# yzqin/s4g-release

Measured on AMD Instinct MI355X. Metric: scenes/sec (25.6k-pt clouds) end-to-end grasp inference, higher is better.
Workload: dtype f32 (f16x2 split)

## Files before the change

### s4g_release_amd/csrc/mlp_heads.hip

```cpp
#include <stdlib.h>

#include "mlp_common.h"

#ifndef S4G_HEADS_ABLATE
#define S4G_HEADS_ABLATE 0
#endif

namespace s4g {

__device__ __forceinline__ void heads_keep_alive(const f32x16& v) { asm volatile("" ::"v"(v)); }

struct HeadsParams {
  int P, N;
  const float* X;
  int ldx;
  const uint16_t* W[5];
  const float* bias[5];
  const float* wsc[5];
  float* out[4];
  int ch[4];
  long long obs[4];
  int head_mask;
  int sigmoid_head;
  const float* a_amax;
  float a_floor;
  int rps;
  const uint16_t* Wp[2];
  const float* bias_p[2];
  const float* wsc_p[2];
  const int* nidx;
  const float* nw;
  const float* sparse;
  const float* dense;
  const float* lbias;
  const float* a_amax2;
  int N2;
};

template <int PL, int HD_RING, int NRBT, bool PRE>
__global__ __launch_bounds__(512, 2) void mlp_heads_kernel(const HeadsParams p) {
  constexpr int BM = 32 * NRBT, C = 256, NW = 8, astr = C + 8, aplane = BM * astr;
  constexpr int FB = PL * 1024;
  extern __shared__ __attribute__((aligned(16))) float smemf[];
  uint16_t* PA = reinterpret_cast<uint16_t*>(smemf);
  uint16_t* PB = PA + PL * aplane;
  float* scr = reinterpret_cast<float*>(PB + PL * aplane);

  const int t = threadIdx.x;
  const int lane = t & 63;
  const int li = lane & 31, lh = lane >> 5;
  const int wv = __builtin_amdgcn_readfirstlane(t >> 6);
  const int p0 = blockIdx.x * BM;
  const uint32_t wf_lane = (uint32_t)lane * 16u;

  float sa = 1.f, inv_sa = 1.f;
  if constexpr (PL == 2) {
    float amax = p.a_floor;
    if constexpr (PRE) {
      if (p.a_amax) amax += amax_rows(p.a_amax, lane, p0, min(p0 + BM, p.P) - 1, p.rps);
      if (p.a_amax2) amax += amax_rows(p.a_amax2, lane, p0, min(p0 + BM, p.P) - 1, p.rps);
    } else if (p.a_amax) {
      amax = fmaxf(amax, amax_rows(p.a_amax, lane, p0, min(p0 + BM, p.P) - 1, p.rps));
    }
    uint32_t ex = __float_as_uint(amax) >> 23;
    ex = ex < 15u ? 15u : (ex > 240u ? 240u : ex);
    ex = __builtin_amdgcn_readfirstlane(ex);
    sa = __uint_as_float((268u - ex) << 23);
    inv_sa = __uint_as_float((ex - 14u) << 23);
  }

  WRef wrs[5];
#pragma unroll
  for (int L = 0; L < 5; ++L) wrs[L] = wref(p.W[L], 0);
  auto woff = [&](int n32, int nks, int ks) { return (size_t)((n32 * nks + ks) * FB); };
  auto w0 = [&](int g, int h) { return wrs[0] + woff(g * 16 + h * 8 + wv, 16, 0); };
  auto w1 = [&](int g, int h) { return wrs[1] + woff(g * 8 + wv, 32, h * 16); };
  auto w2 = [&](int g) { return wrs[2] + woff(g * 8 + wv, 16, 0); };
  auto w3 = [&](int g) { return wrs[3] + woff(g * 4 + (wv & 3), 16, 0); };
  auto wl = [&](int g) { return wrs[4] + woff(g, 8, 0); };
  auto wload = [&](const WRef& w, uint32_t byte_off, int pl) { return wref_load(w, wf_lane + pl * 1024, byte_off); };
  const WRef wp0 = PRE ? wref(p.Wp[0], woff(wv, 16, 0)) : wrs[0];
  const WRef wp1 = PRE ? wref(p.Wp[1], woff(wv, 16, 0)) : wrs[0];

  const int hmask = p.head_mask;
  const int g_first = __builtin_ctz(hmask);
  uint4 ring[HD_RING][PL];
  {
    const WRef w = PRE ? wp0 : w0(g_first, 0);
#pragma unroll
    for (int d = 0; d < HD_RING; ++d)
#pragma unroll
      for (int pl = 0; pl < PL; ++pl) ring[d][pl] = wload(w, d * FB, pl);
  }

#pragma unroll 1
  for (int r0 = 0; r0 < BM; r0 += 64) {
    const int row = r0 + (t >> 3), chunk = t & 7;
    const bool ok = p0 + row < p.P;
    float4 ra[8];
    if constexpr (PRE) {
      const int pos = ok ? p0 + row : 0;
      const int bq = pos / p.N;
      int i3[3];
      float w3[3];
#pragma unroll
      for (int k = 0; k < 3; ++k) {
        i3[k] = bq * p.N2 + p.nidx[(size_t)pos * 3 + k];
        w3[k] = p.nw[(size_t)pos * 3 + k];
      }
#pragma unroll
      for (int h = 0; h < 2; ++h) {
        float4 a[4], b[4], c[4], y[4], bb[4];
#pragma unroll
        for (int kk = 0; kk < 4; ++kk) {
          const int col = (h * 4 + kk) * 32 + chunk * 4;
          a[kk] = *reinterpret_cast<const float4*>(p.sparse + (size_t)i3[0] * 256 + col);
          b[kk] = *reinterpret_cast<const float4*>(p.sparse + (size_t)i3[1] * 256 + col);
          c[kk] = *reinterpret_cast<const float4*>(p.sparse + (size_t)i3[2] * 256 + col);
          bb[kk] = *reinterpret_cast<const float4*>(p.lbias + col);
          y[kk] = p.dense ? *reinterpret_cast<const float4*>(p.dense + (size_t)pos * 256 + col)
                          : make_float4(0.f, 0.f, 0.f, 0.f);
        }
#pragma unroll
        for (int kk = 0; kk < 4; ++kk) {
          const float av[4] = {a[kk].x, a[kk].y, a[kk].z, a[kk].w}, bv[4] = {b[kk].x, b[kk].y, b[kk].z, b[kk].w};
          const float cv[4] = {c[kk].x, c[kk].y, c[kk].z, c[kk].w}, yv[4] = {y[kk].x, y[kk].y, y[kk].z, y[kk].w};
          const float bi[4] = {bb[kk].x, bb[kk].y, bb[kk].z, bb[kk].w};
          float r[4];
#pragma unroll
          for (int e = 0; e < 4; ++e) {
            float acc = __fmul_rn(av[e], w3[0]);
            acc = __fadd_rn(acc, __fmul_rn(bv[e], w3[1]));
            acc = __fadd_rn(acc, __fmul_rn(cv[e], w3[2]));
            r[e] = ok ? fmaxf(__fadd_rn(__fadd_rn(yv[e], acc), bi[e]), 0.f) : 0.f;
          }
          ra[h * 4 + kk] = make_float4(r[0], r[1], r[2], r[3]);
        }
      }
    } else {
    const float* src = p.X + (size_t)(ok ? p0 + row : 0) * p.ldx + chunk * 4;
#pragma unroll
    for (int kt = 0; kt < 8; ++kt)
      ra[kt] = ok ? nt_load4(src + kt * 32) : make_float4(0.f, 0.f, 0.f, 0.f);
    }
#pragma unroll
    for (int kt = 0; kt < 8; ++kt) {
      uint16_t* dst = PA + row * astr + kt * 32 + chunk * 4;
      if constexpr (PL == 2) {
        uint2 h, l;
        split2_h<false>(ra[kt], sa, h, l);
        *reinterpret_cast<uint2*>(dst) = h;
        *reinterpret_cast<uint2*>(dst + aplane) = l;
      } else {
        *reinterpret_cast<uint2*>(dst) = make_uint2(cvt_pk_bf16(ra[kt].x, ra[kt].y), cvt_pk_bf16(ra[kt].z, ra[kt].w));
      }
    }
  }
  __syncthreads();

#define S4G_HD_TERM(NRB, PA_, PB_, ZERO)                                                            \
  _Pragma("unroll") for (int rb = 0; rb < NRB; ++rb)                                                \
    acc[rb] = chain_mfma<PL>(bf[PB_], af[rb][PA_], (ZERO) ? zero16 : acc[rb]);
#define S4G_HD_STRIP(PANEL, NRB, ROWOFF, WCUR, NKS, WNEXT)                                          \
  {                                                                                                 \
    const uint16_t* a_lane = (PANEL) + ((ROWOFF) + li) * astr + 8 * lh;                             \
    uint4 afn[NRBT][PL];                                                                            \
    _Pragma("unroll") for (int rb = 0; rb < NRB; ++rb) _Pragma("unroll") for (int pl = 0; pl < PL; ++pl) \
      afn[rb][pl] = *reinterpret_cast<const uint4*>(a_lane + pl * aplane + rb * 32 * astr);         \
    const WRef wcur_ = (WCUR);                                                                      \
    const WRef wnext_ = (WNEXT);                                                                    \
    _Pragma("unroll") for (int ks = 0; ks < NKS; ++ks) {                                            \
      const int d = ks % HD_RING;                                                                   \
      const int ksn = ks + 1 == NKS ? 0 : ks + 1;                                                   \
      uint4 af[NRBT][PL], bf[PL];                                                                   \
      _Pragma("unroll") for (int rb = 0; rb < NRB; ++rb) _Pragma("unroll") for (int pl = 0; pl < PL; ++pl) { \
        af[rb][pl] = afn[rb][pl];                                                                   \
        if (!(S4G_HEADS_ABLATE & 2))                                                                \
          afn[rb][pl] = *reinterpret_cast<const uint4*>(a_lane + pl * aplane + rb * 32 * astr + ksn * 16); \
      }                                                                                             \
      _Pragma("unroll") for (int pl = 0; pl < PL; ++pl) bf[pl] = ring[d][pl];                       \
      {                                                                                             \
        const int kr = ks + HD_RING;                                                                \
        _Pragma("unroll") for (int pl = 0; pl < PL; ++pl)                                           \
          if (!(S4G_HEADS_ABLATE & 1))                                                              \
            ring[d][pl] = kr < NKS ? wload(wcur_, kr * FB, pl) : wload(wnext_, (kr - NKS) * FB, pl); \
      }                                                                                             \
      if constexpr (PL == 2) {                                                                      \
        S4G_HD_TERM(NRB, 0, 1, ks == 0)                                                             \
        S4G_HD_TERM(NRB, 1, 0, false)                                                               \
        S4G_HD_TERM(NRB, 0, 0, false)                                                               \
      } else {                                                                                      \
        S4G_HD_TERM(NRB, 0, 0, ks == 0)                                                             \
      }                                                                                             \
      _Pragma("unroll") for (int q = 0; q < PL; ++q) {                                              \
        __builtin_amdgcn_sched_group_barrier(0x008, 1, 0);                                          \
        __builtin_amdgcn_sched_group_barrier(0x020, 1, 0);                                          \
        __builtin_amdgcn_sched_group_barrier(0x008, 1, 0);                                          \
        __builtin_amdgcn_sched_group_barrier(0x100, 1, 0);                                          \
      }                                                                                             \
      __builtin_amdgcn_sched_barrier(0);                                                            \
    }                                                                                               \
  }

  f32x16 zero16;
#pragma unroll
  for (int r = 0; r < 16; ++r) zero16[r] = 0.f;
  f32x16 acc[NRBT];
  float* epi_s = scr + wv * 64;

  auto stage_sb2 = [&](const float* wsc, const float* bias, int gch, float mul) {
    epi_s[lane] = lane < 32 ? (PL == 2 ? mul * wsc[gch + lane] : 1.f) : bias[gch + lane - 32];
  };
  auto stage_sb = [&](int L, int gch, float mul) { stage_sb2(p.wsc[L], p.bias[L], gch, mul); };

  float inv_sh = 1.f;
  auto panel_epilogue_to = [&](uint16_t* PD, auto nrb_tag, int rowoff, int pch0) {
    constexpr int NRB = decltype(nrb_tag)::value;
    if (S4G_HEADS_ABLATE & 4) {
#pragma unroll
      for (int rb = 0; rb < NRB; ++rb) heads_keep_alive(acc[rb]);
      if (!(S4G_HEADS_ABLATE & 8)) {
        __syncthreads();
        __syncthreads();
      }
      return;
    }
    float tmax = 0.f;
#pragma unroll
    for (int j = 0; j < 4; ++j) {
      const float4 sc4 = *reinterpret_cast<const float4*>(epi_s + 8 * j + 4 * lh);
      const float4 b4 = *reinterpret_cast<const float4*>(epi_s + 32 + 8 * j + 4 * lh);
      const float scv[4] = {sc4.x, sc4.y, sc4.z, sc4.w};
      const float bv[4] = {b4.x, b4.y, b4.z, b4.w};
#pragma unroll
      for (int rb = 0; rb < NRB; ++rb) {
        const f32x2 x01 = pk_fma(f32x2{acc[rb][4 * j], acc[rb][4 * j + 1]}, f32x2{scv[0], scv[1]}, f32x2{bv[0], bv[1]});
        const f32x2 x23 = pk_fma(f32x2{acc[rb][4 * j + 2], acc[rb][4 * j + 3]}, f32x2{scv[2], scv[3]}, f32x2{bv[2], bv[3]});
        const float x[4] = {fmaxf(x01.x, 0.f), fmaxf(x01.y, 0.f), fmaxf(x23.x, 0.f), fmaxf(x23.y, 0.f)};
#pragma unroll
        for (int e = 0; e < 4; ++e) acc[rb][4 * j + e] = x[e];
        if constexpr (PL == 2) {
          tmax = fmaxf(fmaxf(tmax, x[0]), x[1]);
          tmax = fmaxf(fmaxf(tmax, x[2]), x[3]);
        }
      }
    }
    float sh = 1.f;
    if constexpr (PL == 2) {
      const uint32_t wm = wave_max_u32(__float_as_uint(tmax));
      if (lane == 0) scr[NW * 64 + wv] = __uint_as_float(wm);
    }
    __syncthreads();
    if constexpr (PL == 2) {
      float hmax = scr[NW * 64];
#pragma unroll
      for (int w = 1; w < NW; ++w) hmax = fmaxf(hmax, scr[NW * 64 + w]);
      uint32_t exh = __float_as_uint(hmax) >> 23;
      exh = exh < 15u ? 15u : (exh > 240u ? 240u : exh);
      exh = __builtin_amdgcn_readfirstlane(exh);
      sh = __uint_as_float((268u - exh) << 23);
      inv_sh = __uint_as_float((exh - 14u) << 23);
    }
#pragma unroll
    for (int j = 0; j < 4; ++j)
#pragma unroll
      for (int rb = 0; rb < NRB; ++rb) {
        uint16_t* dst = PD + (rowoff + rb * 32 + li) * astr + pch0 + 8 * j + 4 * lh;
        if constexpr (PL == 2) {
          const float4 v = make_float4(acc[rb][4 * j], acc[rb][4 * j + 1], acc[rb][4 * j + 2], acc[rb][4 * j + 3]);
          uint2 h, l;
          split2_h<false>(v, sh, h, l);
          *reinterpret_cast<uint2*>(dst) = h;
          *reinterpret_cast<uint2*>(dst + aplane) = l;
        } else {
          *reinterpret_cast<uint2*>(dst) = make_uint2(cvt_pk_bf16(acc[rb][4 * j], acc[rb][4 * j + 1]),
                                                      cvt_pk_bf16(acc[rb][4 * j + 2], acc[rb][4 * j + 3]));
        }
      }
    __syncthreads();
  };
  auto panel_epilogue = [&](auto nrb_tag, int rowoff, int pch0) { panel_epilogue_to(PB, nrb_tag, rowoff, pch0); };
  using full = std::integral_constant<int, NRBT>;
  using half = std::integral_constant<int, NRBT / 2>;

  if constexpr (PRE) {
    stage_sb2(p.wsc_p[0], p.bias_p[0], wv * 32, inv_sa);
    S4G_HD_STRIP(PA, NRBT, 0, wp0, 16, wp1)
    panel_epilogue(full{}, 0, wv * 32);
    stage_sb2(p.wsc_p[1], p.bias_p[1], wv * 32, inv_sh);
    S4G_HD_STRIP(PB, NRBT, 0, wp1, 16, w0(g_first, 0))
    panel_epilogue_to(PA, full{}, 0, wv * 32);
    inv_sa = inv_sh;
  }

  for (int g = g_first, gn; g >= 0; g = gn) {
    const int rest = hmask >> (g + 1);
    gn = rest ? g + 1 + __builtin_ctz(rest) : -1;
    const int gnx = gn >= 0 ? gn : g;
    f32x16 acc1[NRBT];
    stage_sb(0, g * 512 + wv * 32, inv_sa);
    S4G_HD_STRIP(PA, NRBT, 0, w0(g, 0), 16, w1(g, 0))
    panel_epilogue(full{}, 0, wv * 32);
    S4G_HD_STRIP(PB, NRBT, 0, w1(g, 0), 16, w0(g, 1))
#pragma unroll
    for (int rb = 0; rb < NRBT; ++rb)
#pragma unroll
      for (int r = 0; r < 16; r += 2) {
        const f32x2 v = f32x2{acc[rb][r], acc[rb][r + 1]} * f32x2{inv_sh, inv_sh};
        acc1[rb][r] = v.x;
        acc1[rb][r + 1] = v.y;
      }
    stage_sb(0, g * 512 + 256 + wv * 32, inv_sa);
    S4G_HD_STRIP(PA, NRBT, 0, w0(g, 1), 16, w1(g, 1))
    panel_epilogue(full{}, 0, wv * 32);
    S4G_HD_STRIP(PB, NRBT, 0, w1(g, 1), 16, w2(g))
#pragma unroll
    for (int rb = 0; rb < NRBT; ++rb)
#pragma unroll
      for (int r = 0; r < 16; r += 2) {
        const f32x2 v = pk_fma(f32x2{acc[rb][r], acc[rb][r + 1]}, f32x2{inv_sh, inv_sh}, f32x2{acc1[rb][r], acc1[rb][r + 1]});
        acc[rb][r] = v.x;
        acc[rb][r + 1] = v.y;
      }
    stage_sb(1, g * 256 + wv * 32, 1.f);
    panel_epilogue(full{}, 0, wv * 32);
    stage_sb(2, g * 256 + wv * 32, inv_sh);
    S4G_HD_STRIP(PB, NRBT, 0, w2(g), 16, w3(g))
    panel_epilogue(full{}, 0, wv * 32);
    {
      const int row3 = (wv >> 2) * (BM / 2), cg = wv & 3;
      stage_sb(3, g * 128 + cg * 32, inv_sh);
      const WRef after = wv < NRBT ? wl(g) : w0(gnx, 0);
      S4G_HD_STRIP(PB, NRBT / 2, row3, w3(g), 16, after)
      panel_epilogue(half{}, row3, cg * 32);
    }
    if (wv < NRBT) {
      stage_sb(4, g * 32, inv_sh);
      S4G_HD_STRIP(PB, 1, wv * 32, wl(g), 8, w0(gnx, 0))
      const int row = p0 + wv * 32 + li;
      const int b = row / p.N, pt = row - b * p.N;
      const int nch = p.ch[g];
      float* __restrict__ base = p.out[g] + (size_t)b * (size_t)p.obs[g] + pt;
#pragma unroll
      for (int j = 0; j < 4; ++j) {
        const float4 sc4 = *reinterpret_cast<const float4*>(epi_s + 8 * j + 4 * lh);
        const float4 b4 = *reinterpret_cast<const float4*>(epi_s + 32 + 8 * j + 4 * lh);
        const float scv[4] = {sc4.x, sc4.y, sc4.z, sc4.w};
        const float bv[4] = {b4.x, b4.y, b4.z, b4.w};
#pragma unroll
        for (int e = 0; e < 4; ++e) {
          const int c = 8 * j + 4 * lh + e;
          float x = __fmaf_rn(acc[0][4 * j + e], scv[e], bv[e]);
          if (g == p.sigmoid_head) x = 1.0f / (1.0f + expf(-x));
          if (c < nch && row < p.P) base[(size_t)c * p.N] = x;
        }
      }
    }
  }
#undef S4G_HD_STRIP
#undef S4G_HD_TERM
}

template <int PL, int HD_RING, int NRBT, bool PRE>
static int launch_heads_cfg(const HeadsParams& p, hipStream_t st) {
  constexpr int BM = 32 * NRBT;
  constexpr size_t lds = sizeof(uint16_t) * 2 * PL * BM * (256 + 8) + sizeof(float) * (8 * 64 + 16);
  static_assert(lds <= 160 * 1024, "one workgroup's panels must fit a CU's LDS");
  static LdsAttrCache lds_cache;
  if (int rc = allow_dynamic_lds(reinterpret_cast<const void*>(&mlp_heads_kernel<PL, HD_RING, NRBT, PRE>), lds, lds_cache)) return rc;
  hipLaunchKernelGGL((mlp_heads_kernel<PL, HD_RING, NRBT, PRE>), dim3((unsigned)((p.P + BM - 1) / BM)), dim3(512), lds, st, p);
  S4G_LAUNCH_CHECK();
  return S4G_OK;
}
template <int PL, int HD_RING, int NRBT>
static int launch_heads(const HeadsParams& p, hipStream_t st) {
  return p.Wp[0] ? launch_heads_cfg<PL, HD_RING, NRBT, true>(p, st) : launch_heads_cfg<PL, HD_RING, NRBT, false>(p, st);
}

}

extern "C" int s4g_heads_chain_f32(const s4g_heads_desc_t* d, s4g_stream_t stream) {
  using namespace s4g;
  if (!d || d->P < 0 || d->N <= 0) return S4G_EINVAL;
  const bool pre = d->pre_W_frag[0] != nullptr;
  if (!pre && (!d->X || (d->ldx & 3) || d->ldx < 256 || ((uintptr_t)d->X & 15))) return S4G_EINVAL;
  if (pre && (!d->pre_W_frag[1] || !d->pre_bias[0] || !d->pre_bias[1] || !d->pre_nidx || !d->pre_nw ||
              !d->pre_sparse || !d->pre_lbias || d->pre_N2 < 3 || ((uintptr_t)d->pre_sparse & 15) ||
              ((uintptr_t)d->pre_dense & 15) || ((uintptr_t)d->pre_lbias & 15) ||
              (d->precision == S4G_GEMM_F16X2 && (!d->pre_w_inv_scale[0] || !d->pre_w_inv_scale[1]))))
    return S4G_EINVAL;
  if (d->precision != S4G_GEMM_F16X2 && d->precision != S4G_GEMM_BF16) return S4G_EINVAL;
  if (d->C != 256 || d->H0 != 512 || d->H1 != 256 || d->H2 != 256 || d->H3 != 128) return S4G_EUNSUPPORTED;
  HeadsParams p;
  p.P = d->P;
  p.N = d->N;
  p.X = d->X;
  p.ldx = d->ldx;
  for (int l = 0; l < 5; ++l) {
    if (!d->W_frag[l] || !d->bias[l] || (d->precision == S4G_GEMM_F16X2 && !d->w_inv_scale[l])) return S4G_EINVAL;
    p.W[l] = (const uint16_t*)d->W_frag[l];
    p.bias[l] = d->bias[l];
    p.wsc[l] = d->w_inv_scale[l];
  }
  p.head_mask = d->head_mask ? d->head_mask : 15;
  if (p.head_mask < 0 || p.head_mask > 15) return S4G_EINVAL;
  for (int h = 0; h < 4; ++h) {
    p.out[h] = nullptr;
    p.ch[h] = 0;
    p.obs[h] = 0;
    if (!((p.head_mask >> h) & 1)) continue;
    if (!d->out[h] || d->channels[h] <= 0 || d->channels[h] > 32) return S4G_EINVAL;
    p.out[h] = d->out[h];
    p.ch[h] = d->channels[h];
    if (d->out_batch_stride != 0 && d->out_batch_stride < (int64_t)d->channels[h] * d->N) return S4G_EINVAL;
    p.obs[h] = d->out_batch_stride != 0 ? (long long)d->out_batch_stride : (long long)d->channels[h] * d->N;
  }
  p.sigmoid_head = d->sigmoid_head;
  p.a_amax = d->a_amax;
  p.a_floor = d->a_amax_floor;
  p.rps = d->rows_per_scene > 0 ? d->rows_per_scene : 0;
  for (int l = 0; l < 2; ++l) {
    p.Wp[l] = pre ? (const uint16_t*)d->pre_W_frag[l] : nullptr;
    p.bias_p[l] = pre ? d->pre_bias[l] : nullptr;
    p.wsc_p[l] = pre ? d->pre_w_inv_scale[l] : nullptr;
  }
  p.nidx = pre ? d->pre_nidx : nullptr;
  p.nw = pre ? d->pre_nw : nullptr;
  p.sparse = pre ? d->pre_sparse : nullptr;
  p.dense = pre ? d->pre_dense : nullptr;
  p.lbias = pre ? d->pre_lbias : nullptr;
  p.a_amax2 = pre ? d->pre_a_amax2 : nullptr;
  p.N2 = pre ? d->pre_N2 : 0;
  if (d->precision == S4G_GEMM_F16X2 && !d->a_amax && !(d->a_amax_floor > 0.f)) return S4G_EINVAL;
  if (d->P == 0) return S4G_OK;
  hipStream_t st = (hipStream_t)stream;
  if (d->precision == S4G_GEMM_F16X2) return launch_heads<2, 4, 2>(p, st);
  return launch_heads<1, 4, 4>(p, st);
}
```

Measured before the change: 2074.

## Make MLP heads kernel persistent with atomic tile queue and next-tile prefetch

Turns the heads kernel into a persistent kernel launched with one workgroup per CU, where workgroups pull tiles from a global atomic queue kept in a per-stream slot and reset by the last workgroup to finish. On the last head of each tile, the f16x2 NRBT=2 path prefetches the next tile's interpolated input and amax scale, staging it into the LDS A panel while the remaining GEMM strips run. This is meant to hide the input gather and split latency behind MFMA work and to cut per-workgroup launch and prologue overhead. In exchange it adds host-side slot bookkeeping (mutex, graph-capture handling), more register pressure, and correctness risk from the queue reset.

```diff
diff --git a/s4g_release_amd/csrc/mlp_heads.hip b/s4g_release_amd/csrc/mlp_heads.hip
--- a/s4g_release_amd/csrc/mlp_heads.hip
+++ b/s4g_release_amd/csrc/mlp_heads.hip
@@ -1,4 +1,6 @@
 #include <stdlib.h>
+
+#include <mutex>
 
 #include "mlp_common.h"
 
@@ -35,39 +37,73 @@
   const float* lbias;
   const float* a_amax2;
   int N2;
+  int ntiles, qslot;
 };
 
-template <int PL, int HD_RING, int NRBT, bool PRE>
+constexpr int HQ_EAGER = 64, HQ_SLOTS = 256;
+__device__ unsigned int g_heads_queue[HQ_SLOTS][2];
+
+#ifdef S4G_HEADS_STAMPS
+__device__ unsigned long long g_heads_stamps[512 * 8];
+#define S4G_HSTAMP(i)                                                                              \
+  do {                                                                                             \
+    const unsigned sb_ = p.ntiles >= 1024 ? (unsigned)(tile - p.ntiles / 2) : (unsigned)tile;      \
+    if (threadIdx.x == 0 && sb_ < 512u) g_heads_stamps[sb_ * 8 + (i)] = __builtin_amdgcn_s_memtime(); \
+  } while (0)
+#else
+#define S4G_HSTAMP(i)
+#endif
+
+template <int PL, int HD_RING, int NRBT, bool PRE, bool PERSIST>
 __global__ __launch_bounds__(512, 2) void mlp_heads_kernel(const HeadsParams p) {
   constexpr int BM = 32 * NRBT, C = 256, NW = 8, astr = C + 8, aplane = BM * astr;
+  constexpr bool PF = PERSIST && PL == 2 && NRBT == 2;
   constexpr int FB = PL * 1024;
   extern __shared__ __attribute__((aligned(16))) float smemf[];
   uint16_t* PA = reinterpret_cast<uint16_t*>(smemf);
   uint16_t* PB = PA + PL * aplane;
   float* scr = reinterpret_cast<float*>(PB + PL * aplane);
+  int* tile_s = reinterpret_cast<int*>(scr + NW * 64 + 8);
+  float* lb_s = scr + NW * 64 + 16;
 
   const int t = threadIdx.x;
   const int lane = t & 63;
   const int li = lane & 31, lh = lane >> 5;
   const int wv = __builtin_amdgcn_readfirstlane(t >> 6);
-  const int p0 = blockIdx.x * BM;
   const uint32_t wf_lane = (uint32_t)lane * 16u;
 
-  float sa = 1.f, inv_sa = 1.f;
-  if constexpr (PL == 2) {
+  auto fetch_tile = [&]() {
+    if (t == 0) tile_s[0] = (int)atomicAdd(&g_heads_queue[p.qslot][0], 1u);
+  };
+  int tile = blockIdx.x;
+  if constexpr (PERSIST) {
+    fetch_tile();
+    if constexpr (PF && PRE) {
+      if (t < 256) lb_s[t] = p.lbias[t];
+    }
+    __syncthreads();
+    tile = __builtin_amdgcn_readfirstlane(tile_s[0]);
+  }
+  if (!PERSIST || tile < p.ntiles) {
+  int p0 = tile * BM;
+
+  auto tile_exp = [&](int q0, bool pre, float va, float vb) -> uint32_t {
     float amax = p.a_floor;
+    const int q1 = min(q0 + BM, p.P) - 1;
+    auto rows = [&](const float* slots, float v) {
+      return pre ? __uint_as_float(wave_max_u32(__float_as_uint(v))) : amax_rows(slots, lane, q0, q1, p.rps);
+    };
     if constexpr (PRE) {
-      if (p.a_amax) amax += amax_rows(p.a_amax, lane, p0, min(p0 + BM, p.P) - 1, p.rps);
-      if (p.a_amax2) amax += amax_rows(p.a_amax2, lane, p0, min(p0 + BM, p.P) - 1, p.rps);
+      if (p.a_amax) amax += rows(p.a_amax, va);
+      if (p.a_amax2) amax += rows(p.a_amax2, vb);
     } else if (p.a_amax) {
-      amax = fmaxf(amax, amax_rows(p.a_amax, lane, p0, min(p0 + BM, p.P) - 1, p.rps));
+      amax = fmaxf(amax, rows(p.a_amax, va));
     }
     uint32_t ex = __float_as_uint(amax) >> 23;
     ex = ex < 15u ? 15u : (ex > 240u ? 240u : ex);
-    ex = __builtin_amdgcn_readfirstlane(ex);
-    sa = __uint_as_float((268u - ex) << 23);
-    inv_sa = __uint_as_float((ex - 14u) << 23);
-  }
+    return __builtin_amdgcn_readfirstlane(ex);
+  };
+  float sa = 1.f, inv_sa = 1.f;
 
   WRef wrs[5];
 #pragma unroll
@@ -84,18 +120,47 @@
 
   const int hmask = p.head_mask;
   const int g_first = __builtin_ctz(hmask);
+  const WRef w_first = PRE ? wp0 : w0(g_first, 0);
   uint4 ring[HD_RING][PL];
-  {
-    const WRef w = PRE ? wp0 : w0(g_first, 0);
-#pragma unroll
-    for (int d = 0; d < HD_RING; ++d)
-#pragma unroll
-      for (int pl = 0; pl < PL; ++pl) ring[d][pl] = wload(w, d * FB, pl);
-  }
+
+  auto interp4 = [&](const float4 a, const float4 b, const float4 c, const float4 y, const float4 bb, const float (&w3)[3], bool ok) {
+    const float av[4] = {a.x, a.y, a.z, a.w}, bv[4] = {b.x, b.y, b.z, b.w};
+    const float cv[4] = {c.x, c.y, c.z, c.w}, yv[4] = {y.x, y.y, y.z, y.w};
+    const float bi[4] = {bb.x, bb.y, bb.z, bb.w};
+    float r[4];
+#pragma unroll
+    for (int e = 0; e < 4; ++e) {
+      float acc = __fmul_rn(av[e], w3[0]);
+      acc = __fadd_rn(acc, __fmul_rn(bv[e], w3[1]));
+      acc = __fadd_rn(acc, __fmul_rn(cv[e], w3[2]));
+      r[e] = ok ? fmaxf(__fadd_rn(__fadd_rn(yv[e], acc), bi[e]), 0.f) : 0.f;
+    }
+    return make_float4(r[0], r[1], r[2], r[3]);
+  };
+
+  auto in_loop = [](int v) {
+    asm volatile("" : "+v"(v));
+    return v;
+  };
+  bool have_x = false;
+  float inv_sa_n = 1.f;
+  for (;;) {
+  S4G_HSTAMP(0);
+  if (!PF || !have_x) {
+  if constexpr (PL == 2) {
+    const uint32_t ex = tile_exp(p0, false, 0.f, 0.f);
+    sa = __uint_as_float((268u - ex) << 23);
+    inv_sa = __uint_as_float((ex - 14u) << 23);
+  }
+#pragma unroll
+  for (int d = 0; d < HD_RING; ++d)
+#pragma unroll
+    for (int pl = 0; pl < PL; ++pl) ring[d][pl] = wload(w_first, d * FB, pl);
 
 #pragma unroll 1
   for (int r0 = 0; r0 < BM; r0 += 64) {
-    const int row = r0 + (t >> 3), chunk = t & 7;
+    const int tp = PERSIST ? in_loop(t) : t;
+    const int row = r0 + (tp >> 3), chunk = tp & 7;
     const bool ok = p0 + row < p.P;
     float4 ra[8];
     if constexpr (PRE) {
@@ -122,20 +187,7 @@
                           : make_float4(0.f, 0.f, 0.f, 0.f);
         }
 #pragma unroll
-        for (int kk = 0; kk < 4; ++kk) {
-          const float av[4] = {a[kk].x, a[kk].y, a[kk].z, a[kk].w}, bv[4] = {b[kk].x, b[kk].y, b[kk].z, b[kk].w};
-          const float cv[4] = {c[kk].x, c[kk].y, c[kk].z, c[kk].w}, yv[4] = {y[kk].x, y[kk].y, y[kk].z, y[kk].w};
-          const float bi[4] = {bb[kk].x, bb[kk].y, bb[kk].z, bb[kk].w};
-          float r[4];
-#pragma unroll
-          for (int e = 0; e < 4; ++e) {
-            float acc = __fmul_rn(av[e], w3[0]);
-            acc = __fadd_rn(acc, __fmul_rn(bv[e], w3[1]));
-            acc = __fadd_rn(acc, __fmul_rn(cv[e], w3[2]));
-            r[e] = ok ? fmaxf(__fadd_rn(__fadd_rn(yv[e], acc), bi[e]), 0.f) : 0.f;
-          }
-          ra[h * 4 + kk] = make_float4(r[0], r[1], r[2], r[3]);
-        }
+        for (int kk = 0; kk < 4; ++kk) ra[h * 4 + kk] = interp4(a[kk], b[kk], c[kk], y[kk], bb[kk], w3, ok);
       }
     } else {
     const float* src = p.X + (size_t)(ok ? p0 + row : 0) * p.ldx + chunk * 4;
@@ -157,6 +209,85 @@
     }
   }
   __syncthreads();
+  } else {
+    inv_sa = inv_sa_n;
+  }
+  S4G_HSTAMP(1);
+
+  int nt = p.ntiles;
+  int n_pos = 0, n_i3[3] = {0, 0, 0};
+  bool n_ok = false, n_one = false;
+  float n_w3[3] = {0.f, 0.f, 0.f}, n_va = 0.f, n_vb = 0.f, n_sa = 1.f;
+  float4 pf[PRE ? 4 : 1][2];
+  auto pf_ids = [&]() {
+    nt = __builtin_amdgcn_readfirstlane(tile_s[0]);
+    if (nt < p.ntiles) {
+      const int q0 = nt * BM, q1 = min(q0 + BM, p.P) - 1;
+      n_ok = q0 + (t >> 3) < p.P;
+      n_pos = n_ok ? q0 + (t >> 3) : 0;
+      const int s0 = p.rps > 0 ? q0 / p.rps : 0, s1 = p.rps > 0 ? q1 / p.rps : 0;
+      n_one = s0 == s1;
+      if (n_one) {
+        if (p.a_amax) n_va = p.a_amax[(size_t)s0 * 64 + lane];
+        if (PRE && p.a_amax2) n_vb = p.a_amax2[(size_t)s0 * 64 + lane];
+      }
+      if constexpr (PRE) {
+#pragma unroll
+        for (int k = 0; k < 3; ++k) {
+          n_i3[k] = p.nidx[(size_t)n_pos * 3 + k];
+          n_w3[k] = p.nw[(size_t)n_pos * 3 + k];
+        }
+      }
+    }
+  };
+  auto pf_load = [&](int q) {
+    if (nt < p.ntiles) {
+      const int chunk = in_loop(t) & 7;
+      if (q == 0) {
+        const uint32_t ex = tile_exp(nt * BM, n_one, n_va, n_vb);
+        n_sa = __uint_as_float((268u - ex) << 23);
+        inv_sa_n = __uint_as_float((ex - 14u) << 23);
+      }
+      if constexpr (PRE) {
+        if (q == 0) {
+          const int bq = n_pos / p.N;
+#pragma unroll
+          for (int k = 0; k < 3; ++k) n_i3[k] += bq * p.N2;
+        }
+#pragma unroll
+        for (int kk = 0; kk < 2; ++kk) {
+          const int col = (q * 2 + kk) * 32 + chunk * 4;
+#pragma unroll
+          for (int k = 0; k < 3; ++k) pf[k][kk] = *reinterpret_cast<const float4*>(p.sparse + (size_t)n_i3[k] * 256 + col);
+          pf[3][kk] = p.dense ? *reinterpret_cast<const float4*>(p.dense + (size_t)n_pos * 256 + col)
+                              : make_float4(0.f, 0.f, 0.f, 0.f);
+        }
+      } else {
+        const float* src = p.X + (size_t)n_pos * p.ldx + chunk * 4;
+#pragma unroll
+        for (int kk = 0; kk < 2; ++kk)
+          pf[0][kk] = n_ok ? nt_load4(src + (q * 2 + kk) * 32) : make_float4(0.f, 0.f, 0.f, 0.f);
+      }
+    }
+  };
+  auto pf_store = [&](int q) {
+    if (nt < p.ntiles) {
+      const int tq = in_loop(t);
+      const int row = tq >> 3, chunk = tq & 7;
+#pragma unroll
+      for (int kk = 0; kk < 2; ++kk) {
+        const int col = (q * 2 + kk) * 32 + chunk * 4;
+        float4 r = pf[0][kk];
+        if constexpr (PRE)
+          r = interp4(pf[0][kk], pf[1][kk], pf[2][kk], pf[3][kk], *reinterpret_cast<const float4*>(lb_s + col), n_w3, n_ok);
+        uint16_t* dst = PA + row * astr + col;
+        uint2 hh, ll;
+        split2_h<false>(r, n_sa, hh, ll);
+        *reinterpret_cast<uint2*>(dst) = hh;
+        *reinterpret_cast<uint2*>(dst + aplane) = ll;
+      }
+    }
+  };
 
 #define S4G_HD_TERM(NRB, PA_, PB_, ZERO)                                                            \
   _Pragma("unroll") for (int rb = 0; rb < NRB; ++rb)                                                \
@@ -297,10 +428,17 @@
     const int rest = hmask >> (g + 1);
     gn = rest ? g + 1 + __builtin_ctz(rest) : -1;
     const int gnx = gn >= 0 ? gn : g;
+    const WRef w_after = PF && gn < 0 ? w_first : w0(gnx, 0);
+    if constexpr (PF) {
+      if (gn < 0) fetch_tile();
+    }
     f32x16 acc1[NRBT];
     stage_sb(0, g * 512 + wv * 32, inv_sa);
     S4G_HD_STRIP(PA, NRBT, 0, w0(g, 0), 16, w1(g, 0))
     panel_epilogue(full{}, 0, wv * 32);
+    if constexpr (PF) {
+      if (gn < 0) pf_ids();
+    }
     S4G_HD_STRIP(PB, NRBT, 0, w1(g, 0), 16, w0(g, 1))
 #pragma unroll
     for (int rb = 0; rb < NRBT; ++rb)
@@ -311,9 +449,24 @@
         acc1[rb][r + 1] = v.y;
       }
     stage_sb(0, g * 512 + 256 + wv * 32, inv_sa);
+    if constexpr (PF) {
+      if (gn < 0) pf_load(0);
+    }
     S4G_HD_STRIP(PA, NRBT, 0, w0(g, 1), 16, w1(g, 1))
     panel_epilogue(full{}, 0, wv * 32);
+    if constexpr (PF) {
+      if (gn < 0) {
+        pf_store(0);
+        pf_load(1);
+      }
+    }
     S4G_HD_STRIP(PB, NRBT, 0, w1(g, 1), 16, w2(g))
+    if constexpr (PF) {
+      if (gn < 0) {
+        pf_store(1);
+        pf_load(2);
+      }
+    }
 #pragma unroll
     for (int rb = 0; rb < NRBT; ++rb)
 #pragma unroll
@@ -326,17 +479,29 @@
     panel_epilogue(full{}, 0, wv * 32);
     stage_sb(2, g * 256 + wv * 32, inv_sh);
     S4G_HD_STRIP(PB, NRBT, 0, w2(g), 16, w3(g))
+    if (gn < 0) { S4G_HSTAMP(2); }
+    if constexpr (PF) {
+      if (gn < 0) {
+        pf_store(2);
+        pf_load(3);
+      }
+    }
     panel_epilogue(full{}, 0, wv * 32);
     {
       const int row3 = (wv >> 2) * (BM / 2), cg = wv & 3;
       stage_sb(3, g * 128 + cg * 32, inv_sh);
-      const WRef after = wv < NRBT ? wl(g) : w0(gnx, 0);
+      const WRef after = wv < NRBT ? wl(g) : w_after;
       S4G_HD_STRIP(PB, NRBT / 2, row3, w3(g), 16, after)
       panel_epilogue(half{}, row3, cg * 32);
+      if constexpr (PF) {
+        if (gn < 0) pf_store(3);
+      }
     }
     if (wv < NRBT) {
+      if (gn < 0) { S4G_HSTAMP(3); }
       stage_sb(4, g * 32, inv_sh);
-      S4G_HD_STRIP(PB, 1, wv * 32, wl(g), 8, w0(gnx, 0))
+      S4G_HD_STRIP(PB, 1, wv * 32, wl(g), 8, w_after)
+      const int lhl = PERSIST ? in_loop(lh) : lh;
       const int row = p0 + wv * 32 + li;
       const int b = row / p.N, pt = row - b * p.N;
       const int nch = p.ch[g];
@@ -349,28 +514,114 @@
         const float bv[4] = {b4.x, b4.y, b4.z, b4.w};
 #pragma unroll
         for (int e = 0; e < 4; ++e) {
-          const int c = 8 * j + 4 * lh + e;
+          const int c = 8 * j + 4 * lhl + e;
           float x = __fmaf_rn(acc[0][4 * j + e], scv[e], bv[e]);
           if (g == p.sigmoid_head) x = 1.0f / (1.0f + expf(-x));
           if (c < nch && row < p.P) base[(size_t)c * p.N] = x;
         }
       }
-    }
+      if (gn < 0) { S4G_HSTAMP(4); }
+    }
+  }
+  S4G_HSTAMP(5);
+  if constexpr (!PERSIST) {
+    break;
+  } else if constexpr (PF) {
+    if (nt >= p.ntiles) break;
+    __syncthreads();
+    tile = nt;
+    have_x = true;
+  } else {
+    fetch_tile();
+    __syncthreads();
+    tile = __builtin_amdgcn_readfirstlane(tile_s[0]);
+    if (tile >= p.ntiles) break;
+  }
+  p0 = tile * BM;
+  }
   }
 #undef S4G_HD_STRIP
 #undef S4G_HD_TERM
-}
-
-template <int PL, int HD_RING, int NRBT, bool PRE>
-static int launch_heads_cfg(const HeadsParams& p, hipStream_t st) {
+  if constexpr (PERSIST) {
+    if (t == 0) {
+      __threadfence();
+      if (atomicAdd(&g_heads_queue[p.qslot][1], 1u) == gridDim.x - 1) {
+        __threadfence();
+        atomicExch(&g_heads_queue[p.qslot][0], 0u);
+        atomicExch(&g_heads_queue[p.qslot][1], 0u);
+      }
+    }
+  }
+}
+
+struct HeadsQueueHost {
+  std::mutex m;
+  hipStream_t streams[HQ_EAGER];
+  int nstreams = 0, ncaptured = 0;
+};
+static int heads_queue_slot(hipStream_t st, int dev) {
+  static HeadsQueueHost host[64];
+  if (dev < 0 || dev >= 64) return -1;
+  hipStreamCaptureStatus cs = hipStreamCaptureStatusNone;
+  if (hipStreamIsCapturing(st, &cs) != hipSuccess) {
+    (void)hipGetLastError();
+    return -1;
+  }
+  HeadsQueueHost& h = host[dev];
+  std::lock_guard<std::mutex> lock(h.m);
+  if (cs != hipStreamCaptureStatusNone) return h.ncaptured < HQ_SLOTS - HQ_EAGER ? HQ_EAGER + h.ncaptured++ : -1;
+  for (int i = 0; i < h.nstreams; ++i)
+    if (h.streams[i] == st) return i;
+  if (h.nstreams == HQ_EAGER) return -1;
+  h.streams[h.nstreams] = st;
+  return h.nstreams++;
+}
+static int heads_cu_count(int dev) {
+  static std::atomic<int> cus[64];
+  const bool slot = dev >= 0 && dev < 64;
+  int n = slot ? cus[dev].load(std::memory_order_relaxed) : 0;
+  if (n > 0) return n;
+  if (hipDeviceGetAttribute(&n, hipDeviceAttributeMultiprocessorCount, dev) != hipSuccess || n <= 0) {
+    (void)hipGetLastError();
+    return 0;
+  }
+  if (slot) cus[dev].store(n, std::memory_order_relaxed);
+  return n;
+}
+
+template <int PL, int HD_RING, int NRBT, bool PRE, bool PERSIST>
+static int launch_heads_form(const HeadsParams& p, unsigned grid, hipStream_t st) {
   constexpr int BM = 32 * NRBT;
-  constexpr size_t lds = sizeof(uint16_t) * 2 * PL * BM * (256 + 8) + sizeof(float) * (8 * 64 + 16);
+  constexpr size_t lds = sizeof(uint16_t) * 2 * PL * BM * (256 + 8) + sizeof(float) * (8 * 64 + 16) +
+                         (PERSIST && PRE && PL == 2 ? sizeof(float) * 256 : 0);
   static_assert(lds <= 160 * 1024, "one workgroup's panels must fit a CU's LDS");
   static LdsAttrCache lds_cache;
-  if (int rc = allow_dynamic_lds(reinterpret_cast<const void*>(&mlp_heads_kernel<PL, HD_RING, NRBT, PRE>), lds, lds_cache)) return rc;
-  hipLaunchKernelGGL((mlp_heads_kernel<PL, HD_RING, NRBT, PRE>), dim3((unsigned)((p.P + BM - 1) / BM)), dim3(512), lds, st, p);
+  if (int rc = allow_dynamic_lds(reinterpret_cast<const void*>(&mlp_heads_kernel<PL, HD_RING, NRBT, PRE, PERSIST>), lds, lds_cache)) return rc;
+  hipLaunchKernelGGL((mlp_heads_kernel<PL, HD_RING, NRBT, PRE, PERSIST>), dim3(grid), dim3(512), lds, st, p);
   S4G_LAUNCH_CHECK();
   return S4G_OK;
+}
+template <int PL, int HD_RING, int NRBT, bool PRE>
+static int launch_heads_cfg(const HeadsParams& p0, hipStream_t st) {
+  constexpr int BM = 32 * NRBT;
+  HeadsParams p = p0;
+  p.ntiles = (p.P + BM - 1) / BM;
+  p.qslot = 0;
+  int dev = 0;
+  if (hipError_t e = hipGetDevice(&dev); e != hipSuccess) return (int)e;
+  int wgs = 0;
+  if (const char* k = knob("S4G_HEADS_WGS")) {
+    wgs = atoi(k);
+    if (wgs < 0 || wgs > 65535) return S4G_EINVAL;
+  } else if (PL == 2) {
+    const int cus = heads_cu_count(dev);
+    if (cus > 0 && p.ntiles > cus) wgs = cus;
+  }
+  if (wgs > 0) {
+    p.qslot = heads_queue_slot(st, dev);
+    if (p.qslot >= 0) return launch_heads_form<PL, HD_RING, NRBT, PRE, true>(p, (unsigned)wgs, st);
+  }
+  return launch_heads_form<PL, HD_RING, NRBT, PRE, false>(p, (unsigned)p.ntiles, st);
 }
 template <int PL, int HD_RING, int NRBT>
 static int launch_heads(const HeadsParams& p, hipStream_t st) {
@@ -378,6 +629,12 @@
 }
 
 }
+
+#ifdef S4G_HEADS_STAMPS
+extern "C" int s4g_debug_heads_stamps(unsigned long long* host_out_512x8) {
+  return (int)hipMemcpyFromSymbol(host_out_512x8, HIP_SYMBOL(s4g::g_heads_stamps), sizeof(unsigned long long) * 512 * 8);
+}
+#endif
 
 extern "C" int s4g_heads_chain_f32(const s4g_heads_desc_t* d, s4g_stream_t stream) {
   using namespace s4g;
```

After: 2093, median of 6. No clear change (+1.0%).
